# fkluger/vanishing_points_2017

Measured on AMD Instinct MI355X. Metric: images/sec (LSD->CNN->EM) + horizon-AUC parity, YUD-shape, 1/2/4/8 GPU, higher is better.
Workload: dtype f32 (CNN: f32 operands / accumulation / results; conv1 multiply EXACT bf16 pieces of the f32 operands (three per operand) on the bf16 matrix cores; conv2-5, fc6 and fc7 multiply scaled fp16 PAIRS of the f32 operands (22 of 24 significand bits, three exact products per f32 product) on the fp16 matrix

## Files before the change

vanishing_points_2017_amd/csrc/em_run.hpp:

```cpp
#ifndef VPK_EM_RUN_HPP_
#define VPK_EM_RUN_HPP_

#include "em_ctx.hpp"
#include "em_linalg.hpp"
#include "em_setup.hpp"
#include "em_estep.hpp"
#include "em_smooth.hpp"
#include "em_assign.hpp"
#include "em_mstep.hpp"
#include "em_vpset.hpp"

namespace vpk {

struct EmOut {
    double* vp;
    double* sigma;
    double* counts;
    double* counts_w;
    int* num_vp;
    long long* assoc;
    int* iterations;
    int* status;
    unsigned* flags;
    double* metric;
// ... 63 lines not shown
        *o.status = status;
        *o.flags = sh.flags;
    }
    block_sync();
}

VPK_DEV void trace_put(EmOut& o, int i, int slot, double v) {
    if (o.trace && tid() == 0) o.trace[TRACE_COLS * i + slot] = v;
}
VPK_DEV void trace_add(EmOut& o, int i, int slot, double v) {
    if (o.trace && tid() == 0) o.trace[TRACE_COLS * i + slot] += v;
}


constexpr int EM_DONE = 0, EM_SUSPENDED = 1;
constexpr long long EM_NO_DEADLINE = 0x7fffffffffffffffll;
struct EmSlice {
    long long deadline;
    int start_iter;
};

VPK_DEVFN void save_state(EmCtx& c) {
    typedef VPK_GLOBAL unsigned long long* gup;
    gup dst = (gup)c.state;
    const unsigned long long* src = reinterpret_cast<const unsigned long long*>(&SH());
    for (int q = tid(); q < (int)(sizeof(Shared) / 8); q += nthreads()) dst[q] = src[q];
    block_sync();
}
VPK_DEVFN void restore_state(EmCtx& c) {
    typedef const VPK_GLOBAL unsigned long long* cgup;
    cgup src = (cgup)c.state;
    unsigned long long* dst = reinterpret_cast<unsigned long long*>(&SH());
    block_sync();
    for (int q = tid(); q < (int)(sizeof(Shared) / 8); q += nthreads()) dst[q] = src[q];
    block_sync();
}

template <int MEASURE = VPK_DIST_ANGLE>
VPK_DEVFN int em_run(EmCtx& c, EmOut& o, EmSlice& sl) {
    static_assert(MEASURE == VPK_DIST_ANGLE || MEASURE == VPK_DIST_DOTPROD, "the EM runs \"angle\" and \"dotprod\" (vp_localisation.py:196-203)");
    Shared& sh = SH();
    const vpk_em_params& P = c.prm;
    const double max_stdd = MEASURE == VPK_DIST_DOTPROD ? 1e-3 : 1e-6;
    const double merge_thresh_final = P.merge_thresh * 10;
    const int split_merge_it = 100;
    long long tk = clock_ticks();
    const long long t_begin = tk;
    int first = 0;
    bool ew_valid = false;
    if (sl.start_iter >= 0) {
        restore_state(c);
        first = sl.start_iter;
    } else {
    if (tid() == 0) { sh.flags = 0; sh.M = 0; sh.ncomp = 0; sh.ibuf[5] = 0; sh.ibuf[2] = 0; sh.active_us = 0; for (int q = 8; q < 16; ++q) sh.dbuf[q] = 0; }
    block_sync();
    if (o.trace)
        for (int q = tid(); q < TRACE_COLS * (P.num_iter + 1); q += nthreads()) o.trace[q] = 0.0;
    if (c.N <= 0) { write_result(c, o, VPK_EM_NO_VP, 0); return EM_DONE; }

    if (P.use_weights) { pairwise_setup(c, true); zero_tail_rows(c); }
    else pairwise_setup(c, false);
    trace_put(o, P.num_iter, 0, lap(tk));
    normalise_lines(c);
    for (int q = tid(); q < 3 * c.N; q += nthreads()) c.lcopy[q] = c.l[q];
    for (int q = tid(); q < 4 * c.N; q += nthreads()) c.lpcopy[q] = c.lp[q];
    block_sync();
    c.l = c.lcopy;
    c.lp = c.lpcopy;
    initial_vps(c);
    const int m_found = sh.M;
    prior_setup(c);
    if (m_found == 0) { write_result(c, o, VPK_EM_NO_INITIAL_VP, 0); return EM_DONE; }
    if (c.init_vp) {
        if (tid() == 0) {
            int m = c.n_init < MAXM ? c.n_init : MAXM;
            for (int k = 0; k < m; ++k) {
                cgdp q = c.init_vp + 3 * (size_t)k;
                double nr = norm3(q[0], q[1], q[2]);
                sh.cur[3 * k] = q[0] / nr; sh.cur[3 * k + 1] = q[1] / nr; sh.cur[3 * k + 2] = q[2] / nr;
            }
            sh.M = m;
        }
        block_sync();
    }
    weights_setup(c);
    line_geometry_setup<MEASURE>(c);
    for (int m = tid(); m < MAXM; m += nthreads()) {
        sh.s[m] = 1.0 * (sh.sigma_prior * max_stdd);
        sh.nxt[3 * m] = 0; sh.nxt[3 * m + 1] = 0; sh.nxt[3 * m + 2] = 0;
    }
    block_sync();

    estep<MEASURE>(c, sh.cur);
    smooth(c);
    assign_lines<MEASURE>(c, true);
    count_lines(c);
    const int m_initial = sh.M;
    for (int m = tid(); m < sh.M; m += nthreads()) sh.removed[m] = sh.cnt[m] < 3;
    block_sync();
    compact_vps(c);
    ew_valid = c.smoother != 1 && sh.M == m_initial;
    trace_put(o, P.num_iter, 1, lap(tk));
    }

    for (int i = first; i < P.num_iter; ++i) {
        if (sl.deadline != EM_NO_DEADLINE && i > sl.start_iter) {
            if (tid() == 0) sh.ibuf[6] = clock_ticks() >= sl.deadline;
            block_sync();
            if (sh.ibuf[6]) {
                if (tid() == 0) sh.active_us += (double)(clock_ticks() - t_begin) * CLOCK_US;
                block_sync();
                save_state(c);
                sl.start_iter = i;
                return EM_SUSPENDED;
            }
        }
        tk = clock_ticks();
        const long long t_iter = tk;
        if (sh.M == 0) { write_result(c, o, VPK_EM_NO_VP, 0); return EM_DONE; }
        double events = 0;
        bool ew_skip = ew_valid;
        ew_valid = false;
        if (i % P.split_merge_freq == 0 && i > 0 && i < split_merge_it && P.do_split) {
            int mb = sh.M;
// ... 111 lines not shown
```

vanishing_points_2017_amd/csrc/em_setup.hpp:

```cpp
#ifndef VPK_EM_SETUP_HPP_
#define VPK_EM_SETUP_HPP_

#include "em_ctx.hpp"

namespace vpk {

VPK_DEVFN void normalise_lines(EmCtx& c) {
    for (int n = tid(); n < c.N; n += nthreads()) {
        gdp r = c.l + 3 * (size_t)n;
        for (int pass = 0; pass < 2; ++pass) {
            double nr = norm3(r[0], r[1], r[2]);
            r[0] /= nr; r[1] /= nr; r[2] /= nr;
        }
    }
    block_sync();
}

constexpr int PW_TILED_MIN = 512;
constexpr int PW_RB = 16;
constexpr int PW_TLD = WAVE + 1;
constexpr int PW_TBUF = 2 * PW_RB * PW_TLD;
VPK_DEV void pairwise_tiles(EmCtx& c) {
    const int N = c.N;
    double* gs = SCRATCH() + wave_id() * (PW_RB * 10);
    static_assert(8 * PW_RB * 10 <= PART_DOUBLES, "row geometries of eight waves in the setup scratch");
    const bool tbuf_ok = WAVE == 64 && PART_DOUBLES + nwaves() * PW_TBUF <= c.wt_doubles;
    double* tb = SCRATCH() + PART_DOUBLES + wave_id() * PW_TBUF;
    const int nb = (N + PW_RB - 1) / PW_RB;
    int t = 0;
    for (int I = 0; I < nb; ++I) {
        const int i0 = I * PW_RB;
        const int ilast = (i0 + PW_RB < N ? i0 + PW_RB : N) - 1;
        const int nch = (ilast + WAVE - 1) / WAVE;
        for (int jc = 0; jc < nch; ++jc, ++t) {
            if (t % nwaves() != wave_id()) continue;
            if (lane() < PW_RB) {
                const int i = i0 + lane() < N ? i0 + lane() : N - 1;
                double a[4];
#pragma unroll
                for (int q = 0; q < 4; ++q) a[q] = c.lp[4 * (size_t)i + q];
                const LineGeom g = line_geom(a);
                double* o = gs + lane() * 10;
                o[0] = g.x1; o[1] = g.y1; o[2] = g.x2; o[3] = g.y2; o[4] = g.dx; o[5] = g.dy; o[6] = g.nn; o[7] = g.vx; o[8] = g.vy; o[9] = g.nv;
            }
            wave_lds_order();
            const int j = jc * WAVE + lane();
            const int jj = j < N ? j : N - 1;
            double b[4];
#pragma unroll
            for (int q = 0; q < 4; ++q) b[q] = c.lp[4 * (size_t)jj + q];
            const LineGeom gb = line_geom(b);
            auto row_geom = [&](int r) {
                const double* o = gs + r * 10;
                LineGeom g;
                g.x1 = o[0]; g.y1 = o[1]; g.x2 = o[2]; g.y2 = o[3]; g.dx = o[4]; g.dy = o[5]; g.nn = o[6]; g.vx = o[7]; g.vy = o[8]; g.nv = o[9];
                return g;
            };
            auto put = [&](int i, double d, double sim) {
                if (!(j < i && i < N)) return;
                c.lsim[(size_t)i * c.ld + j] = sim;
                c.lsim[(size_t)j * c.ld + i] = sim;
                c.pdist[(size_t)i * c.ld + j] = d;
                c.pdist[(size_t)j * c.ld + i] = d;
            };
            const bool interior = tbuf_ok && jc * WAVE + WAVE - 1 < i0 && i0 + PW_RB <= N;
            for (int r = 0; r < PW_RB; r += 2) {
                const LineGeom g0 = row_geom(r), g1 = row_geom(r + 1);
                const double d0 = line_distance_closest(g0, gb);
                const double d1 = line_distance_closest(g1, gb);
                const double s0 = lines_cosangle(g0, gb, 9.0) * proximity(d0, g0.nv, gb.nv, 1.0);
                const double s1 = lines_cosangle(g1, gb, 9.0) * proximity(d1, g1.nv, gb.nv, 1.0);
                if (interior) {
                    c.lsim[(size_t)(i0 + r) * c.ld + j] = s0;   c.pdist[(size_t)(i0 + r) * c.ld + j] = d0;
                    c.lsim[(size_t)(i0 + r + 1) * c.ld + j] = s1; c.pdist[(size_t)(i0 + r + 1) * c.ld + j] = d1;
                    tb[r * PW_TLD + lane()] = s0;               tb[(PW_RB + r) * PW_TLD + lane()] = d0;
                    tb[(r + 1) * PW_TLD + lane()] = s1;         tb[(PW_RB + r + 1) * PW_TLD + lane()] = d1;
                } else {
                    put(i0 + r, d0, s0);
                    put(i0 + r + 1, d1, s1);
                }
            }
            wave_lds_order();
            if (interior) {
                const int cp = lane() & 7, jr = lane() >> 3;
#pragma unroll
                for (int q = 0; q < 8; ++q) {
                    const int jl = 8 * q + jr;
                    const size_t at = (size_t)(jc * WAVE + jl) * c.ld + i0 + 2 * cp;
                    store_cols2(c.lsim + at, tb[(2 * cp) * PW_TLD + jl], tb[(2 * cp + 1) * PW_TLD + jl]);
                    store_cols2(c.pdist + at, tb[(PW_RB + 2 * cp) * PW_TLD + jl], tb[(PW_RB + 2 * cp + 1) * PW_TLD + jl]);
                }
                wave_lds_order();
            }
        }
    }
    for (int i = tid(); i < N; i += nthreads()) {
        c.lsim[(size_t)i * c.ld + i] = 0.0;
        c.pdist[(size_t)i * c.ld + i] = 4.0;
    }
}

VPK_DEVFN void pairwise_setup(EmCtx& c, bool want_lsim) {
    const int N = c.N;
    if (want_lsim) {
        if (N >= PW_TILED_MIN && WAVE == 64 && c.smoother != 1) pairwise_tiles(c);
        else
        for (int r = wave_id(); 2 * r < N; r += nwaves()) {
            const int i0 = r, i1 = N - 1 - r;
            const int len = i0 == i1 ? i0 : i0 + i1;
            double a0[4], a1[4];
#pragma unroll
            for (int q = 0; q < 4; ++q) { a0[q] = c.lp[4 * (size_t)i0 + q]; a1[q] = c.lp[4 * (size_t)i1 + q]; }
            const LineGeom g0 = line_geom(a0), g1 = line_geom(a1);
            auto one = [&](int t, double& d, double& sim) {
                const bool first = t < i0;
                const int j = t < len ? (first ? t : t - i0) : 0;
                const LineGeom& ga = first ? g0 : g1;
                double b[4] = {c.lp[4 * (size_t)j], c.lp[4 * (size_t)j + 1], c.lp[4 * (size_t)j + 2], c.lp[4 * (size_t)j + 3]};
                const LineGeom gb = line_geom(b);
                d = line_distance_closest(ga, gb);
                sim = lines_cosangle(ga, gb, 9.0) * proximity(d, ga.nv, gb.nv, 1.0);
            };
            auto put = [&](int t, double d, double sim) {
                if (t >= len) return;
                const int i = t < i0 ? i0 : i1, j = t < i0 ? t : t - i0;
                c.lsim[(size_t)i * c.ld + j] = sim;
                c.lsim[(size_t)j * c.ld + i] = sim;
                c.pdist[(size_t)i * c.ld + j] = d;
                c.pdist[(size_t)j * c.ld + i] = d;
            };
            for (int t = lane(); t < len; t += 2 * WAVE) {
                double d0, s0, d1, s1;
                one(t, d0, s0);
                one(t + WAVE, d1, s1);
                put(t, d0, s0);
                put(t + WAVE, d1, s1);
            }
            if (lane() == 0) {
                c.lsim[(size_t)i0 * c.ld + i0] = 0.0;
                c.pdist[(size_t)i0 * c.ld + i0] = 4.0;
                c.lsim[(size_t)i1 * c.ld + i1] = 0.0;
                c.pdist[(size_t)i1 * c.ld + i1] = 4.0;
            }
        }
        block_sync();
        for (int i = wave_id(); i < N; i += nwaves()) {
            cgdp srow = c.lsim + (size_t)i * c.ld;
            double rsum = 0.0;
            for (int j = lane(); j < N; j += WAVE) rsum += srow[j];
            rsum = wave_sum(rsum);
            if (lane() == 0) c.rowsum[i] = rsum;
        }
        constexpr int RPW = WAVE / ROWG;
        const int grp = lane() / ROWG, gl = lane() % ROWG;
        const int k1 = N < KNN1 ? N : KNN1;
        const int k2 = N < KNN2 ? N : KNN2;
        double* ks = SCRATCH() + (wave_id() * RPW + grp) * (4 * KNN1 + KNN2);
        for (int base = wave_id() * RPW; base < N; base += nwaves() * RPW) {
            const int i = base + grp;
            const bool valid = i < N;
            const int ii = valid ? i : 0;
            double td[KNN1];
            int tj[KNN1];
#pragma unroll
            for (int q = 0; q < KNN1; ++q) { td[q] = 1e300; tj[q] = 0x7fffffff; }
            cgdp drow = c.pdist + (size_t)ii * c.ld;
            for (int j0 = gl; j0 < N; j0 += 4 * ROWG) {
                double dv[4];
#pragma unroll
                for (int u = 0; u < 4; ++u) dv[u] = (j0 + u * ROWG < N) ? drow[j0 + u * ROWG] : 1e300;
#pragma unroll
                for (int u = 0; u < 4; ++u) {
                    double nd = dv[u];
                    int nj = (j0 + u * ROWG < N) ? j0 + u * ROWG : 0x7fffffff;
#pragma unroll
                    for (int q = 0; q < KNN1; ++q) {
                        const bool lt = (nd < td[q]) || (nd == td[q] && nj < tj[q]);
                        const double od = td[q];
                        const int oj = tj[q];
                        td[q] = lt ? nd : od;
                        tj[q] = lt ? nj : oj;
                        nd = lt ? od : nd;
                        nj = lt ? oj : nj;
                    }
                }
            }
            for (int r = 0; r < k1; ++r) {
                double bd = td[0];
                int bj = tj[0];
                row16_argmin(bd, bj);
                if (tj[0] == bj && td[0] == bd) {
#pragma unroll
                    for (int q = 0; q + 1 < KNN1; ++q) { td[q] = td[q + 1]; tj[q] = tj[q + 1]; }
                    td[KNN1 - 1] = 1e300;
                    tj[KNN1 - 1] = 0x7fffffff;
                }
                if (gl == 0) { ks[r] = (double)bj; ks[KNN1 + r] = bd; }
            }
            wave_sync();
            double a[4] = {c.lp[4 * (size_t)ii], c.lp[4 * (size_t)ii + 1], c.lp[4 * (size_t)ii + 2], c.lp[4 * (size_t)ii + 3]};
            const double len_a = norm2(a[0] - a[2], a[1] - a[3]);
            for (int q = gl; q < k1; q += ROWG) {
                int j = (int)ks[q];
                j = (valid && j >= 0 && j < N) ? j : 0;
                double b[4] = {c.lp[4 * (size_t)j], c.lp[4 * (size_t)j + 1], c.lp[4 * (size_t)j + 2], c.lp[4 * (size_t)j + 3]};
                ks[2 * KNN1 + q] = lines_cosangle(a, b, 9.0);
                const double dq = j == ii ? line_distance_closest(a, b) : ks[KNN1 + q];
                ks[3 * KNN1 + q] = proximity(dq, len_a, line_length(b), 1.0);
            }
            wave_sync();
            for (int q = gl; q < k1; q += ROWG) {
                const double cq = ks[2 * KNN1 + q];
                int rank = 0;
                for (int p = 0; p < k1; ++p) {
                    const double cp = ks[2 * KNN1 + p];
                    rank += (cp > cq) || (cp == cq && p > q);
                }
                if (rank < k2) ks[4 * KNN1 + rank] = ks[3 * KNN1 + q] * cq;
            }
            wave_sync();
            if (gl == 0 && valid) {
                double sum = 0.0;
                for (int r = 0; r < k2; ++r) sum += ks[4 * KNN1 + r];
                c.lscore[i] = sum / k2;
                c.langle[i] = line_angle(a);
            }
            wave_sync();
        }
        block_sync();
        return;
    }
    double* ks = SCRATCH() + wave_id() * (4 * KNN1 + KNN2);
    const int k1 = N < KNN1 ? N : KNN1;
    const int k2 = N < KNN2 ? N : KNN2;
    for (int i = wave_id(); i < N; i += nwaves()) {
        double a[4] = {c.lp[4 * (size_t)i], c.lp[4 * (size_t)i + 1], c.lp[4 * (size_t)i + 2],
                       c.lp[4 * (size_t)i + 3]};
        const LineGeom ga = line_geom(a);
        const double len_a = ga.nv;
        double rsum = 0.0;
        double td[KNN1];
        int tj[KNN1];
#pragma unroll
        for (int q = 0; q < KNN1; ++q) { td[q] = 1e300; tj[q] = 0x7fffffff; }
        auto pair_eval = [&](int j, double& d, double& sim) {
            const int jj = j < N ? j : i;
            double b[4] = {c.lp[4 * (size_t)jj], c.lp[4 * (size_t)jj + 1], c.lp[4 * (size_t)jj + 2],
                           c.lp[4 * (size_t)jj + 3]};
            const LineGeom gb = line_geom(b);
            d = line_distance_closest(ga, gb);
            sim = want_lsim ? lines_cosangle(ga, gb, 9.0) * proximity(d, len_a, gb.nv, 1.0) : 0.0;
        };
        auto pair_commit = [&](int j, double d, double sim) {
            if (j >= N) return;
            if (want_lsim) {
                sim = (i == j) ? 0.0 : sim;
                c.lsim[(size_t)i * c.ld + j] = sim;
                rsum += sim;
            }
            double nd = (i == j) ? 4.0 : d;
            int nj = j;
#pragma unroll
            for (int q = 0; q < KNN1; ++q) {
                const bool lt = (nd < td[q]) || (nd == td[q] && nj < tj[q]);
                const double od = td[q];
                const int oj = tj[q];
                td[q] = lt ? nd : od;
                tj[q] = lt ? nj : oj;
                nd = lt ? od : nd;
                nj = lt ? oj : nj;
            }
        };
        for (int j = lane(); j < N; j += 2 * WAVE) {
            double d0, s0, d1, s1;
            pair_eval(j, d0, s0);
            pair_eval(j + WAVE, d1, s1);
            pair_commit(j, d0, s0);
            pair_commit(j + WAVE, d1, s1);
        }
        rsum = wave_sum(rsum);
        if (lane() == 0) c.rowsum[i] = rsum;
        for (int r = 0; r < k1; ++r) {
// ... 9 lines not shown
            if (lane() == 0) { ks[r] = (double)bj; ks[KNN1 + r] = bd; }
        }
        wave_sync();
        for (int q = lane(); q < k1; q += WAVE) {
            int j = (int)ks[q];
            double b[4] = {c.lp[4 * (size_t)j], c.lp[4 * (size_t)j + 1], c.lp[4 * (size_t)j + 2],
                           c.lp[4 * (size_t)j + 3]};
            ks[2 * KNN1 + q] = lines_cosangle(a, b, 9.0);
            const double dq = j == i ? line_distance_closest(a, b) : ks[KNN1 + q];
            ks[3 * KNN1 + q] = proximity(dq, len_a, line_length(b), 1.0);
        }
        wave_sync();
        for (int q = lane(); q < k1; q += WAVE) {
            const double cq = ks[2 * KNN1 + q];
            int rank = 0;
            for (int p = 0; p < k1; ++p) {
                const double cp = ks[2 * KNN1 + p];
                rank += (cp > cq) || (cp == cq && p > q);
            }
            if (rank < k2) ks[4 * KNN1 + rank] = ks[3 * KNN1 + q] * cq;
        }
        wave_sync();
        if (lane() == 0) {
            double sum = 0.0;
            for (int r = 0; r < k2; ++r) sum += ks[4 * KNN1 + r];
            c.lscore[i] = sum / k2;
            c.langle[i] = line_angle(a);
        }
        wave_sync();
    }
    block_sync();
}

VPK_DEVFN void weights_setup(EmCtx& c) {
    const int N = c.N;
    const bool uw = c.prm.use_weights != 0;
    for (int n = tid(); n < N; n += nthreads()) {
        double a[4] = {c.lp[4 * (size_t)n], c.lp[4 * (size_t)n + 1], c.lp[4 * (size_t)n + 2],
                       c.lp[4 * (size_t)n + 3]};
        c.lweight[n] = uw ? line_length(a) * clip(c.lscore[n], 0.2, 1.0) : 1.0;
    }
    block_sync();
    for (int k = tid(); k < N; k += nthreads()) {
        c.den[k] = 1 + c.prm.wbias * c.lweight[k] * (uw ? c.rowsum[k] : 0.0);
        if (uw && !(fabs(c.rowsum[k]) <= 1.7976931348623157e308)) SH().ibuf[2] = 1;
    }
    block_sync();
}

VPK_DEVFN void prior_setup(EmCtx& c) {
    Shared& sh = SH();
    float* keep = (float*)SCRATCH();
    if (tid() == 0) sh.sigma_prior = PI_D / (1.282 * GRIDN);
    prior_keep_sum(c.cnn, sh.wts, keep);
    {
        const float sum = keep[NCELL];
        const float dv = prior_norm_f32(sh.sigma_prior);
        int* wcount = (int*)(SCRATCH() + 256);
        for (int base = 0; base < NCELL; base += nthreads()) {
            const int i = base + tid();
            float w = 0.f;
            if (i < NCELL) w = prior_weight(keep[i], sum, dv);
            const unsigned long long pos = wave_ballot(i < NCELL && w > 0);
            if (lane() == 0) wcount[wave_id()] = popcount64(pos);
            block_sync();
            int before = (base == 0) ? 0 : sh.ncomp;
            for (int k = 0; k < wave_id(); ++k) before += wcount[k];
            const int nc = before + popcount64(pos & lanes_below());
            if (i < NCELL) {
                sh.wts[i] = w;
                if (w > 0 && nc < MAXCOMP) {
                    sh.pma[nc] = grid_centre(i % GRIDN);
                    sh.pmb[nc] = grid_centre(i / GRIDN);
                    sh.pw[nc] = (double)w;
                }
            }
            block_sync();
            if (tid() == 0) {
                int tot = before;
                for (int k = 0; k < nwaves(); ++k) tot += wcount[k];
                sh.ncomp = tot < MAXCOMP ? tot : MAXCOMP;
            }
            block_sync();
        }
    }
}

VPK_DEVFN void initial_vps(EmCtx& c) {
    Shared& sh = SH();
    cgfp r = c.cnn;
    for (int i = tid(); i < NCELL; i += nthreads()) {
        int b = i / GRIDN, a = i % GRIDN;
        float vm = r[i];
        float vu = (a + 1 < GRIDN) ? r[b * GRIDN + a + 1] : 0.f;
        float vd = (a - 1 > 0) ? r[b * GRIDN + a - 1] : 0.f;
        float vl = (b - 1 > 0) ? r[(b - 1) * GRIDN + a] : 0.f;
        float vr = (b + 1 < GRIDN) ? r[(b + 1) * GRIDN + a] : 0.f;
        sh.mx[i] = (vm > vu && vm > vd && vm > vl && vm > vr) ? 1 : 0;
    }
    block_sync();
    unsigned char* keep = (unsigned char*)SCRATCH();
    double* cand = SCRATCH() + 64;
    const int num_max = c.prm.num_init_vp;
    for (int i = tid(); i < NCELL; i += nthreads()) {
        int k = 0;
        if (sh.mx[i]) {
            int rank = 0;
            float vi = r[i];
            for (int j = 0; j < NCELL; ++j)
                if (sh.mx[j]) rank += (r[j] > vi) || (r[j] == vi && j > i);
            k = rank < num_max;
        }
        keep[i] = (unsigned char)k;
        cand[4 * i + 3] = 0.0;
    }
    block_sync();
    const int S = c.ssize;
    for (int cell = wave_id(); cell < NCELL; cell += nwaves()) {
        if (!keep[cell]) continue;
        int ra = cell / GRIDN, rb = cell % GRIDN;
        int r0 = ra * S / GRIDN, r1 = (ra + 1) * S / GRIDN;
        int c0 = rb * S / GRIDN, c1 = (rb + 1) * S / GRIDN;
        int bw = c1 - c0, npix = (r1 - r0) * bw;
        constexpr int PV = 10;
        int mxv = 0, cntp = 0, sr = 0, sc = 0;
        if (npix <= PV * WAVE) {
            int vals[PV];
#pragma unroll
            for (int q = 0; q < PV; ++q) {
                const int p = lane() + q * WAVE;
                const int pc = p < npix ? p : 0;
                const int v = c.sphere[(size_t)(S - 1 - (r0 + pc / bw)) * S + c0 + pc % bw];
                vals[q] = p < npix ? v : -1;
            }
#pragma unroll
            for (int q = 0; q < PV; ++q) mxv = vals[q] > mxv ? vals[q] : mxv;
            mxv = wave_max_int(mxv);
            if (mxv == 0) continue;
#pragma unroll
            for (int q = 0; q < PV; ++q) {
                const int p = lane() + q * WAVE;
                if (vals[q] == mxv) { ++cntp; sr += p / bw; sc += p % bw; }
            }
        } else {
            for (int p = lane(); p < npix; p += WAVE) {
                int rr = r0 + p / bw, cc = c0 + p % bw;
                int v = c.sphere[(size_t)(S - 1 - rr) * S + cc];
                mxv = v > mxv ? v : mxv;
            }
            mxv = wave_max_int(mxv);
            if (mxv == 0) continue;
            for (int p = lane(); p < npix; p += WAVE) {
                int rr = p / bw, cc = p % bw;
                int v = c.sphere[(size_t)(S - 1 - (r0 + rr)) * S + c0 + cc];
                if (v == mxv) { ++cntp; sr += rr; sc += cc; }
            }
        }
        cntp = wave_sum_int(cntp);
        sr = wave_sum_int(sr);
        sc = wave_sum_int(sc);
        if (lane() == 0) {
            double avg_r = (double)sr / cntp, avg_c = (double)sc / cntp;
            double ia = avg_c + c0, ib = avg_r + r0;
            double alpha = (ia - 0.5 * S + 0.5) * PI_D / S;
            double beta = (ib - 0.5 * S + 0.5) * PI_D / S;
            double px = sin(alpha) * cos(beta), py = sin(beta), pz = cos(alpha) * cos(beta);
            double sg = sign_np(pz);
            cand[4 * cell + 0] = px * sg;
            cand[4 * cell + 1] = py * sg;
            cand[4 * cell + 2] = pz * sg;
            cand[4 * cell + 3] = 1.0;
        }
    }
    block_sync();
    if (tid() == 0) {
        int m = 0;
        for (int cell = 0; cell < NCELL; ++cell) {
            if (cand[4 * cell + 3] != 0.0 && m < MAXM) {
                sh.cur[3 * m + 0] = cand[4 * cell + 0];
                sh.cur[3 * m + 1] = cand[4 * cell + 1];
                sh.cur[3 * m + 2] = cand[4 * cell + 2];
                ++m;
            }
        }
        sh.M = m;
    }
    block_sync();
}

template <int MEASURE = VPK_DIST_ANGLE>
VPK_DEVFN void line_geometry_setup(EmCtx& c) {
    for (int n = tid(); n < c.N; n += nthreads()) {
        if (MEASURE == VPK_DIST_DOTPROD) {
            cgdp q = c.l + 3 * (size_t)n;
            c.drow[n] = q[0];
            c.drow[(size_t)c.ldn + n] = q[1];
            c.drow[2 * (size_t)c.ldn + n] = q[2];
            continue;
        }
        cgdp q = c.lp + 4 * (size_t)n;
        if (MEASURE == VPK_DIST_AREA) {
            const double mx = 0.5 * (q[0] + q[2]), my = 0.5 * (q[1] + q[3]);
            c.drow[n] = mx;
            c.drow[(size_t)c.ldn + n] = my;
            c.drow[2 * (size_t)c.ldn + n] = q[0];
            c.drow[3 * (size_t)c.ldn + n] = q[1];
            c.drow[4 * (size_t)c.ldn + n] = norm2(mx - q[2], my - q[3]);
            continue;
        }
        const double v2x = q[0] - q[2], v2y = q[1] - q[3];
        c.drow[n] = 0.5 * (q[0] + q[2]);
        c.drow[(size_t)c.ldn + n] = 0.5 * (q[1] + q[3]);
        c.drow[2 * (size_t)c.ldn + n] = v2x;
        c.drow[3 * (size_t)c.ldn + n] = v2y;
        c.drow[4 * (size_t)c.ldn + n] = norm2(v2x, v2y);
    }
    block_sync();
}

}
#endif
```

vanishing_points_2017_amd/csrc/prior_device.hpp:

```cpp
#ifndef VPK_PRIOR_DEVICE_HPP_
#define VPK_PRIOR_DEVICE_HPP_

#include "wave_prims.hpp"

namespace vpk {

constexpr int GRIDN = 20;
constexpr int NCELL = GRIDN * GRIDN;
constexpr int MAXCOMP = 100;
constexpr double PI_D = 3.141592653589793238462643383279502884;

VPK_DEV bool is_nan(double x) { return x != x; }
VPK_DEV double exp_underflow(double x) { return x < -746.0 ? 0.0 : exp(x); }

VPK_DEV void vp_angles(double x0, double x1, double& alpha, double& beta) {
    beta = asin(x1);
    double inner = x0 / cos(beta);
    inner = inner < 1 ? inner : (is_nan(inner) ? inner : 1.0);
    inner = inner > -1 ? inner : (is_nan(inner) ? inner : -1.0);
    alpha = asin(inner);
}

VPK_DEV double mixture_term(double alpha, double beta, double ma, double mb, double kk) {
    double d1 = (alpha - ma) * (alpha - ma) + (beta - mb) * (beta - mb);
    double d2 = (alpha - ma + PI_D) * (alpha - ma + PI_D) + (beta + mb) * (beta + mb);
    double d3 = (alpha - ma - PI_D) * (alpha - ma - PI_D) + (beta + mb) * (beta + mb);
    double d4 = (alpha + ma) * (alpha + ma) + (beta - mb - PI_D) * (beta - mb - PI_D);
    double e4 = exp_underflow(d4 * kk);
    return (((exp_underflow(d1 * kk) + exp_underflow(d2 * kk)) + exp_underflow(d3 * kk)) + e4) + e4;
}

VPK_DEV float np_pairwise_block_f32(const float* a, int n) {
    float r[8];
    for (int j = 0; j < 8; ++j) r[j] = a[j];
    int i;
    for (i = 8; i < n - (n % 8); i += 8)
        for (int j = 0; j < 8; ++j) r[j] += a[i + j];
    float res = ((r[0] + r[1]) + (r[2] + r[3])) + ((r[4] + r[5]) + (r[6] + r[7]));
    for (; i < n; ++i) res += a[i];
    return res;
}
VPK_DEV float np_pairwise_sum_f32_400(const float* a) {
    float lo = np_pairwise_block_f32(a, 96) + np_pairwise_block_f32(a + 96, 104);
    float hi = np_pairwise_block_f32(a + 200, 96) + np_pairwise_block_f32(a + 296, 104);
    return lo + hi;
}

VPK_DEV double grid_centre(int i) {
    double start = -(GRIDN - 1.0) / GRIDN * PI_D / 2;
    double stop = (GRIDN - 1.0) / GRIDN * PI_D / 2;
    double step = (stop - start) / (GRIDN - 1);
    return i == GRIDN - 1 ? stop : i * step + start;
}

VPK_DEV void prior_keep_sum(cgfp cnn, float* wts, float* keep) {
    for (int i = tid(); i < NCELL; i += nthreads()) wts[i] = cnn[i];
    block_sync();
    for (int i = tid(); i < NCELL; i += nthreads()) {
        float wi = wts[i];
        int rank = 0;
        for (int j = 0; j < NCELL; ++j) {
            float wj = wts[j];
            rank += (wj > wi) || (wj == wi && j > i);
        }
        keep[i] = rank < MAXCOMP ? wi : 0.f;
    }
    block_sync();
    if (tid() == 0) keep[NCELL] = np_pairwise_sum_f32_400(keep);
    block_sync();
}
VPK_DEV float prior_norm_f32(double sigma) { return (float)(2 * PI_D * sigma * sigma); }
VPK_DEV float prior_weight(float kept, float sum, float dv) {
    float w = kept / sum;
    return w / dv;
}

constexpr int PRIOR_TILE = WAVE;
constexpr int PRIOR_CHUNK = 128;
constexpr size_t PRIOR_LDS_BYTES = 3 * PRIOR_CHUNK * sizeof(double);

struct MixtureArgs {
    int ncomp, npts;
    cgdp means;
    long long means_stride;
    cgdp weights;
    double kk;
    cgdp pts;
    long long pts_stride;
    gdp angles_out;
    gdp pdf_out;
};

template <int DIM> VPK_DEV void mixture_pdf_tile(const MixtureArgs& a, int b, int t) {
    double* sma = reinterpret_cast<double*>(lds_base());
    double* smb = sma + PRIOR_CHUNK;
    double* sw = smb + PRIOR_CHUNK;
    const int i = t * PRIOR_TILE + tid();
    const bool live = i < a.npts;
    double alpha = 0.0, beta = 0.0;
    if (live) {
        cgdp p = a.pts + (size_t)b * a.pts_stride + (size_t)i * DIM;
        if (DIM == 3) vp_angles(p[0], p[1], alpha, beta);
        else { alpha = p[0]; beta = p[1]; }
    }
    cgdp mean = a.means + (size_t)b * a.means_stride;
    cgdp wt = a.weights + (size_t)b * a.ncomp;
    double acc = 0.0;
    for (int c0 = 0; c0 < a.ncomp; c0 += PRIOR_CHUNK) {
        const int nc = a.ncomp - c0 < PRIOR_CHUNK ? a.ncomp - c0 : PRIOR_CHUNK;
        block_sync();
        for (int q = tid(); q < nc; q += nthreads()) {
            sma[q] = mean[2 * (size_t)(c0 + q)];
            smb[q] = mean[2 * (size_t)(c0 + q) + 1];
            sw[q] = wt[c0 + q];
        }
        block_sync();
        if (live)
            for (int q = 0; q < nc; ++q) {
                const double w = sw[q];
                if (!(w > 0)) continue;
                acc += mixture_term(alpha, beta, sma[q], smb[q], a.kk) * w;
// ... 14 lines not shown
```

Before: 22970.

## Parallelise EM setup: threshold kNN, tabled line geometry, block-parallel initial VPs

```diff
diff --git a/vanishing_points_2017_amd/csrc/em_knn.hpp b/vanishing_points_2017_amd/csrc/em_knn.hpp
--- /dev/null
+++ b/vanishing_points_2017_amd/csrc/em_knn.hpp
@@ -0,0 +1,62 @@
+#ifndef VPK_EM_KNN_HPP_
+#define VPK_EM_KNN_HPP_
+
+#ifndef VPK_DEV
+#define VPK_DEV static inline
+#endif
+
+namespace vpk {
+namespace knn {
+
+constexpr double SENT_D = 1e300;
+constexpr int SENT_J = 0x7fffffff;
+constexpr int CAP = 28;
+constexpr int CAND_DOUBLES = CAP + CAP / 2;
+
+VPK_DEV bool key_less(double ad, int aj, double bd, int bj) { return (ad < bd) || (ad == bd && aj < bj); }
+
+VPK_DEV void key_of(double d, int j, int n, double& kd, int& kj) {
+    const bool ok = j < n && d <= SENT_D;
+    kd = ok ? d : SENT_D;
+    kj = ok ? j : SENT_J;
+}
+
+struct Top2 {
+    double d0, d1;
+    int j0, j1;
+};
+VPK_DEV void top2_init(Top2& t) { t.d0 = t.d1 = SENT_D; t.j0 = t.j1 = SENT_J; }
+VPK_DEV void top2_push(Top2& t, double kd, int kj) {
+    const bool lt0 = key_less(kd, kj, t.d0, t.j0);
+    const bool lt1 = key_less(kd, kj, t.d1, t.j1);
+    t.d1 = lt0 ? t.d0 : (lt1 ? kd : t.d1);
+    t.j1 = lt0 ? t.j0 : (lt1 ? kj : t.j1);
+    t.d0 = lt0 ? kd : t.d0;
+    t.j0 = lt0 ? kj : t.j0;
+}
+VPK_DEV void top2_pop_if(Top2& t, double bd, int bj) {
+    const bool won = t.j0 == bj && t.d0 == bd;
+    t.d0 = won ? t.d1 : t.d0;
+    t.j0 = won ? t.j1 : t.j0;
+    t.d1 = won ? SENT_D : t.d1;
+    t.j1 = won ? SENT_J : t.j1;
+}
+
+VPK_DEV bool is_candidate(double kd, int kj, double td, int tj) {
+    return kj != SENT_J && !key_less(td, tj, kd, kj);
+}
+VPK_DEV int cand_slot(unsigned bits, int g, int listed) { return listed + __builtin_popcount(bits & ((1u << g) - 1u)); }
+
+VPK_DEV void rank_and_place(int g, int G, int cnt, const double* cd, const int* cj, int k, double* out_j, double* out_d) {
+    for (int q = g; q < cnt; q += G) {
+        const double dq = cd[q];
+        const int jq = cj[q];
+        int rank = 0;
+        for (int p = 0; p < cnt; ++p) rank += key_less(cd[p], cj[p], dq, jq) ? 1 : 0;
+        if (rank < k) { out_j[rank] = (double)jq; out_d[rank] = dq; }
+    }
+}
+
+}
+}
+#endif
diff --git a/vanishing_points_2017_amd/csrc/em_run.hpp b/vanishing_points_2017_amd/csrc/em_run.hpp
--- a/vanishing_points_2017_amd/csrc/em_run.hpp
+++ b/vanishing_points_2017_amd/csrc/em_run.hpp
@@ -139,7 +139,7 @@
         restore_state(c);
         first = sl.start_iter;
     } else {
-    if (tid() == 0) { sh.flags = 0; sh.M = 0; sh.ncomp = 0; sh.ibuf[5] = 0; sh.ibuf[2] = 0; sh.active_us = 0; for (int q = 8; q < 16; ++q) sh.dbuf[q] = 0; }
+    if (tid() == 0) { sh.flags = 0; sh.M = 0; sh.ncomp = 0; sh.ibuf[5] = 0; sh.ibuf[2] = 0; sh.active_us = 0; sh.dbuf[0] = 0; sh.dbuf[1] = 0; for (int q = 8; q < 16; ++q) sh.dbuf[q] = 0; }
     block_sync();
     if (o.trace)
         for (int q = tid(); q < TRACE_COLS * (P.num_iter + 1); q += nthreads()) o.trace[q] = 0.0;
@@ -148,15 +148,20 @@
     if (P.use_weights) { pairwise_setup(c, true); zero_tail_rows(c); }
     else pairwise_setup(c, false);
     trace_put(o, P.num_iter, 0, lap(tk));
+    trace_put(o, P.num_iter, 10, sh.dbuf[0]);
+    trace_put(o, P.num_iter, 11, sh.dbuf[1]);
     normalise_lines(c);
     for (int q = tid(); q < 3 * c.N; q += nthreads()) c.lcopy[q] = c.l[q];
     for (int q = tid(); q < 4 * c.N; q += nthreads()) c.lpcopy[q] = c.lp[q];
     block_sync();
     c.l = c.lcopy;
     c.lp = c.lpcopy;
+    long long tq = clock_ticks();
     initial_vps(c);
+    trace_put(o, 0, 8, lap(tq));
     const int m_found = sh.M;
     prior_setup(c);
+    trace_put(o, 0, 9, lap(tq));
     if (m_found == 0) { write_result(c, o, VPK_EM_NO_INITIAL_VP, 0); return EM_DONE; }
     if (c.init_vp) {
         if (tid() == 0) {
diff --git a/vanishing_points_2017_amd/csrc/em_setup.hpp b/vanishing_points_2017_amd/csrc/em_setup.hpp
--- a/vanishing_points_2017_amd/csrc/em_setup.hpp
+++ b/vanishing_points_2017_amd/csrc/em_setup.hpp
@@ -2,6 +2,7 @@
 #define VPK_EM_SETUP_HPP_
 
 #include "em_ctx.hpp"
+#include "em_knn.hpp"
 
 namespace vpk {
 
@@ -100,11 +101,181 @@
     }
 }
 
+template <bool B> struct BoolTag { static constexpr bool value = B; };
+VPK_DEV LineGeom line_geom_known(const double a[4], double nn, double nv) {
+    LineGeom g;
+    g.x1 = a[0]; g.y1 = a[1]; g.x2 = a[2]; g.y2 = a[3];
+    g.dx = a[2] - a[0]; g.dy = a[3] - a[1];
+    g.nn = nn;
+    g.vx = a[0] - a[2]; g.vy = a[1] - a[3];
+    g.nv = nv;
+    return g;
+}
+
+VPK_DEV void knn_by_insertion(cgdp drow, int N, int gl, int k1, double* ks) {
+    double td[KNN1];
+    int tj[KNN1];
+#pragma unroll
+    for (int q = 0; q < KNN1; ++q) { td[q] = 1e300; tj[q] = 0x7fffffff; }
+    for (int j0 = gl; j0 < N; j0 += 4 * ROWG) {
+        double dv[4];
+#pragma unroll
+        for (int u = 0; u < 4; ++u) dv[u] = (j0 + u * ROWG < N) ? drow[j0 + u * ROWG] : 1e300;
+#pragma unroll
+        for (int u = 0; u < 4; ++u) {
+            double nd = dv[u];
+            int nj = (j0 + u * ROWG < N) ? j0 + u * ROWG : 0x7fffffff;
+#pragma unroll
+            for (int q = 0; q < KNN1; ++q) {
+                const bool lt = (nd < td[q]) || (nd == td[q] && nj < tj[q]);
+                const double od = td[q];
+                const int oj = tj[q];
+                td[q] = lt ? nd : od;
+                tj[q] = lt ? nj : oj;
+                nd = lt ? od : nd;
+                nj = lt ? oj : nj;
+            }
+        }
+    }
+    for (int r = 0; r < k1; ++r) {
+        double bd = td[0];
+        int bj = tj[0];
+        row16_argmin(bd, bj);
+        if (tj[0] == bj && td[0] == bd) {
+#pragma unroll
+            for (int q = 0; q + 1 < KNN1; ++q) { td[q] = td[q + 1]; tj[q] = tj[q + 1]; }
+            td[KNN1 - 1] = 1e300;
+            tj[KNN1 - 1] = 0x7fffffff;
+        }
+        if (gl == 0) { ks[r] = (double)bj; ks[KNN1 + r] = bd; }
+    }
+}
+
+constexpr int KNN_RPW = WAVE / ROWG;
+constexpr int KS_ROW = 2 * KNN1 + (2 * KNN1 + KNN2 > knn::CAND_DOUBLES ? 2 * KNN1 + KNN2 : knn::CAND_DOUBLES);
+static_assert(WAVE != 64 || 8 * KNN_RPW * KS_ROW <= PART_DOUBLES, "kNN rows of eight waves in the setup scratch");
+VPK_DEV double* knn_row_scratch() { return SCRATCH() + (wave_id() * KNN_RPW + lane() / ROWG) * KS_ROW; }
+VPK_DEV bool knn_by_threshold(cgdp drow, int N, int k1) {
+    const int grp = lane() / ROWG, gl = lane() % ROWG;
+    double* ks = knn_row_scratch();
+    for (int q = gl; q < k1; q += ROWG) { ks[q] = (double)knn::SENT_J; ks[KNN1 + q] = knn::SENT_D; }
+    constexpr int KB = 16;
+    const bool one_trip = N <= KB * ROWG;
+    double dv[KB];
+    knn::Top2 t2;
+    knn::top2_init(t2);
+    for (int jb = 0; jb < N; jb += KB * ROWG) {
+#pragma unroll
+        for (int u = 0; u < KB; ++u) { const int j = jb + u * ROWG + gl; dv[u] = j < N ? drow[j] : knn::SENT_D; }
+#pragma unroll
+        for (int u = 0; u < KB; ++u) {
+            double kd;
+            int kj;
+            knn::key_of(dv[u], jb + u * ROWG + gl, N, kd, kj);
+            knn::top2_push(t2, kd, kj);
+        }
+    }
+    double taud = knn::SENT_D;
+    int tauj = knn::SENT_J;
+    for (int r = 0; r < k1; ++r) {
+        taud = t2.d0;
+        tauj = t2.j0;
+        row16_argmin(taud, tauj);
+        knn::top2_pop_if(t2, taud, tauj);
+    }
+    double* cd = ks + 2 * KNN1;
+    int* cj = (int*)(cd + knn::CAP);
+    int cnt = 0;
+    for (int jb = 0; jb < N; jb += KB * ROWG) {
+        if (!one_trip) {
+#pragma unroll
+            for (int u = 0; u < KB; ++u) { const int j = jb + u * ROWG + gl; dv[u] = j < N ? drow[j] : knn::SENT_D; }
+        }
+#pragma unroll
+        for (int u = 0; u < KB; ++u) {
+            if (jb + u * ROWG >= N) break;
+            double kd;
+            int kj;
+            knn::key_of(dv[u], jb + u * ROWG + gl, N, kd, kj);
+            const bool in = knn::is_candidate(kd, kj, taud, tauj);
+            const unsigned bits = (unsigned)(wave_ballot(in) >> (grp * ROWG)) & ((1u << ROWG) - 1u);
+            const int at = knn::cand_slot(bits, gl, cnt);
+            if (in && at < knn::CAP) { cd[at] = kd; cj[at] = kj; }
+            cnt += popcount64(bits);
+        }
+    }
+    wave_sync();
+    if (cnt > knn::CAP) return false;
+    knn::rank_and_place(gl, ROWG, cnt, cd, cj, k1, ks, ks + KNN1);
+    return true;
+}
+
+VPK_DEV void line_rating_rows(EmCtx& c) {
+    const int N = c.N;
+    constexpr int RPW = KNN_RPW;
+    const int grp = lane() / ROWG, gl = lane() % ROWG;
+    const int k1 = N < KNN1 ? N : KNN1;
+    const int k2 = N < KNN2 ? N : KNN2;
+    double* ks = knn_row_scratch();
+    for (int base = wave_id() * RPW; base < N; base += nwaves() * RPW) {
+        const int i = base + grp;
+        const bool valid = i < N;
+        const int ii = valid ? i : 0;
+        cgdp drow = c.pdist + (size_t)ii * c.ld;
+        const bool insertion = c.smoother == 1 || !knn_by_threshold(drow, N, k1);
+        if (insertion) knn_by_insertion(drow, N, gl, k1, ks);
+        wave_sync();
+        double a[4] = {c.lp[4 * (size_t)ii], c.lp[4 * (size_t)ii + 1], c.lp[4 * (size_t)ii + 2], c.lp[4 * (size_t)ii + 3]};
+        const double len_a = norm2(a[0] - a[2], a[1] - a[3]);
+        for (int q = gl; q < k1; q += ROWG) {
+            int j = (int)ks[q];
+            j = (valid && j >= 0 && j < N) ? j : 0;
+            double b[4] = {c.lp[4 * (size_t)j], c.lp[4 * (size_t)j + 1], c.lp[4 * (size_t)j + 2], c.lp[4 * (size_t)j + 3]};
+            ks[2 * KNN1 + q] = lines_cosangle(a, b, 9.0);
+            const double dq = j == ii ? line_distance_closest(a, b) : ks[KNN1 + q];
+            ks[3 * KNN1 + q] = proximity(dq, len_a, line_length(b), 1.0);
+        }
+        wave_sync();
+        for (int q = gl; q < k1; q += ROWG) {
+            const double cq = ks[2 * KNN1 + q];
+            int rank = 0;
+            for (int p = 0; p < k1; ++p) {
+                const double cp = ks[2 * KNN1 + p];
+                rank += (cp > cq) || (cp == cq && p > q);
+            }
+            if (rank < k2) ks[4 * KNN1 + rank] = ks[3 * KNN1 + q] * cq;
+        }
+        wave_sync();
+        if (gl == 0 && valid) {
+            double sum = 0.0;
+            for (int r = 0; r < k2; ++r) sum += ks[4 * KNN1 + r];
+            c.lscore[i] = sum / k2;
+            c.langle[i] = line_angle(a);
+        }
+        wave_sync();
+    }
+}
+
 VPK_DEVFN void pairwise_setup(EmCtx& c, bool want_lsim) {
     const int N = c.N;
     if (want_lsim) {
+        long long tq_ = clock_ticks();
         if (N >= PW_TILED_MIN && WAVE == 64 && c.smoother != 1) pairwise_tiles(c);
-        else
+        else {
+        const bool geo_lds = c.smoother != 1 && 2 * N <= PART_DOUBLES;
+        double* gnn = SCRATCH();
+        double* gnv = SCRATCH() + N;
+        if (geo_lds) {
+            for (int n = tid(); n < N; n += nthreads()) {
+                double a[4] = {c.lp[4 * (size_t)n], c.lp[4 * (size_t)n + 1], c.lp[4 * (size_t)n + 2], c.lp[4 * (size_t)n + 3]};
+                const LineGeom g = line_geom(a);
+                gnn[n] = g.nn;
+                gnv[n] = g.nv;
+            }
+            block_sync();
+        }
+        auto rows = [&](auto from_table) {
+        constexpr bool TAB = decltype(from_table)::value;
         for (int r = wave_id(); 2 * r < N; r += nwaves()) {
             const int i0 = r, i1 = N - 1 - r;
             const int len = i0 == i1 ? i0 : i0 + i1;
@@ -117,7 +288,7 @@
                 const int j = t < len ? (first ? t : t - i0) : 0;
                 const LineGeom& ga = first ? g0 : g1;
                 double b[4] = {c.lp[4 * (size_t)j], c.lp[4 * (size_t)j + 1], c.lp[4 * (size_t)j + 2], c.lp[4 * (size_t)j + 3]};
-                const LineGeom gb = line_geom(b);
+                const LineGeom gb = TAB ? line_geom_known(b, gnn[j], gnv[j]) : line_geom(b);
                 d = line_distance_closest(ga, gb);
                 sim = lines_cosangle(ga, gb, 9.0) * proximity(d, ga.nv, gb.nv, 1.0);
             };
@@ -143,91 +314,50 @@
                 c.pdist[(size_t)i1 * c.ld + i1] = 4.0;
             }
         }
+        };
+        if (geo_lds) rows(BoolTag<true>());
+        else rows(BoolTag<false>());
+        }
         block_sync();
-        for (int i = wave_id(); i < N; i += nwaves()) {
-            cgdp srow = c.lsim + (size_t)i * c.ld;
-            double rsum = 0.0;
-            for (int j = lane(); j < N; j += WAVE) rsum += srow[j];
-            rsum = wave_sum(rsum);
-            if (lane() == 0) c.rowsum[i] = rsum;
-        }
-        constexpr int RPW = WAVE / ROWG;
-        const int grp = lane() / ROWG, gl = lane() % ROWG;
-        const int k1 = N < KNN1 ? N : KNN1;
-        const int k2 = N < KNN2 ? N : KNN2;
-        double* ks = SCRATCH() + (wave_id() * RPW + grp) * (4 * KNN1 + KNN2);
-        for (int base = wave_id() * RPW; base < N; base += nwaves() * RPW) {
-            const int i = base + grp;
-            const bool valid = i < N;
-            const int ii = valid ? i : 0;
-            double td[KNN1];
-            int tj[KNN1];
-#pragma unroll
-            for (int q = 0; q < KNN1; ++q) { td[q] = 1e300; tj[q] = 0x7fffffff; }
-            cgdp drow = c.pdist + (size_t)ii * c.ld;
-            for (int j0 = gl; j0 < N; j0 += 4 * ROWG) {
-                double dv[4];
-#pragma unroll
-                for (int u = 0; u < 4; ++u) dv[u] = (j0 + u * ROWG < N) ? drow[j0 + u * ROWG] : 1e300;
-#pragma unroll
-                for (int u = 0; u < 4; ++u) {
-                    double nd = dv[u];
-                    int nj = (j0 + u * ROWG < N) ? j0 + u * ROWG : 0x7fffffff;
-#pragma unroll
-                    for (int q = 0; q < KNN1; ++q) {
-                        const bool lt = (nd < td[q]) || (nd == td[q] && nj < tj[q]);
-                        const double od = td[q];
-                        const int oj = tj[q];
-                        td[q] = lt ? nd : od;
-                        tj[q] = lt ? nj : oj;
-                        nd = lt ? od : nd;
-                        nj = lt ? oj : nj;
+        if (tid() == 0) SH().dbuf[0] = lap(tq_);
+        if (c.smoother == 1) {
+            for (int i = wave_id(); i < N; i += nwaves()) {
+                cgdp srow = c.lsim + (size_t)i * c.ld;
+                double rsum = 0.0;
+                for (int j = lane(); j < N; j += WAVE) rsum += srow[j];
+                rsum = wave_sum(rsum);
+                if (lane() == 0) c.rowsum[i] = rsum;
+            }
+        } else {
+            constexpr int RS_ROWS = 4, RS_COLS = 8;
+            for (int i0 = wave_id() * RS_ROWS; i0 < N; i0 += nwaves() * RS_ROWS) {
+                double rs[RS_ROWS];
+#pragma unroll
+                for (int q = 0; q < RS_ROWS; ++q) rs[q] = 0.0;
+                for (int jb = 0; jb < N; jb += RS_COLS * WAVE) {
+                    double v[RS_ROWS][RS_COLS];
+#pragma unroll
+                    for (int q = 0; q < RS_ROWS; ++q) {
+                        cgdp srow = c.lsim + (size_t)(i0 + q < N ? i0 + q : N - 1) * c.ld;
+#pragma unroll
+                        for (int u = 0; u < RS_COLS; ++u) { const int j = jb + u * WAVE + lane(); v[q][u] = j < N ? srow[j] : 0.0; }
                     }
+#pragma unroll
+                    for (int q = 0; q < RS_ROWS; ++q)
+#pragma unroll
+                        for (int u = 0; u < RS_COLS; ++u)
+                            if (jb + u * WAVE + lane() < N) rs[q] += v[q][u];
                 }
-            }
-            for (int r = 0; r < k1; ++r) {
-                double bd = td[0];
-                int bj = tj[0];
-                row16_argmin(bd, bj);
-                if (tj[0] == bj && td[0] == bd) {
-#pragma unroll
-                    for (int q = 0; q + 1 < KNN1; ++q) { td[q] = td[q + 1]; tj[q] = tj[q + 1]; }
-                    td[KNN1 - 1] = 1e300;
-                    tj[KNN1 - 1] = 0x7fffffff;
+#pragma unroll
+                for (int q = 0; q < RS_ROWS; ++q) {
+                    const double rsum = wave_sum(rs[q]);
+                    if (lane() == 0 && i0 + q < N) c.rowsum[i0 + q] = rsum;
                 }
-                if (gl == 0) { ks[r] = (double)bj; ks[KNN1 + r] = bd; }
-            }
-            wave_sync();
-            double a[4] = {c.lp[4 * (size_t)ii], c.lp[4 * (size_t)ii + 1], c.lp[4 * (size_t)ii + 2], c.lp[4 * (size_t)ii + 3]};
-            const double len_a = norm2(a[0] - a[2], a[1] - a[3]);
-            for (int q = gl; q < k1; q += ROWG) {
-                int j = (int)ks[q];
-                j = (valid && j >= 0 && j < N) ? j : 0;
-                double b[4] = {c.lp[4 * (size_t)j], c.lp[4 * (size_t)j + 1], c.lp[4 * (size_t)j + 2], c.lp[4 * (size_t)j + 3]};
-                ks[2 * KNN1 + q] = lines_cosangle(a, b, 9.0);
-                const double dq = j == ii ? line_distance_closest(a, b) : ks[KNN1 + q];
-                ks[3 * KNN1 + q] = proximity(dq, len_a, line_length(b), 1.0);
-            }
-            wave_sync();
-            for (int q = gl; q < k1; q += ROWG) {
-                const double cq = ks[2 * KNN1 + q];
-                int rank = 0;
-                for (int p = 0; p < k1; ++p) {
-                    const double cp = ks[2 * KNN1 + p];
-                    rank += (cp > cq) || (cp == cq && p > q);
-                }
-                if (rank < k2) ks[4 * KNN1 + rank] = ks[3 * KNN1 + q] * cq;
-            }
-            wave_sync();
-            if (gl == 0 && valid) {
-                double sum = 0.0;
-                for (int r = 0; r < k2; ++r) sum += ks[4 * KNN1 + r];
-                c.lscore[i] = sum / k2;
-                c.langle[i] = line_angle(a);
-            }
-            wave_sync();
-        }
+            }
+        }
+        line_rating_rows(c);
         block_sync();
+        if (tid() == 0) SH().dbuf[1] = lap(tq_);
         return;
     }
     double* ks = SCRATCH() + wave_id() * (4 * KNN1 + KNN2);
@@ -343,7 +473,7 @@
     Shared& sh = SH();
     float* keep = (float*)SCRATCH();
     if (tid() == 0) sh.sigma_prior = PI_D / (1.282 * GRIDN);
-    prior_keep_sum(c.cnn, sh.wts, keep);
+    prior_keep_sum(c.cnn, sh.wts, keep, c.smoother == 1);
     {
         const float sum = keep[NCELL];
         const float dv = prior_norm_f32(sh.sigma_prior);
@@ -377,7 +507,64 @@
     }
 }
 
-VPK_DEVFN void initial_vps(EmCtx& c) {
+VPK_DEV void initial_vp_of_cell(EmCtx& c, int cell, double* out) {
+    const int S = c.ssize;
+    int ra = cell / GRIDN, rb = cell % GRIDN;
+    int r0 = ra * S / GRIDN, r1 = (ra + 1) * S / GRIDN;
+    int c0 = rb * S / GRIDN, c1 = (rb + 1) * S / GRIDN;
+    int bw = c1 - c0, npix = (r1 - r0) * bw;
+    constexpr int PV = 10;
+    int mxv = 0, cntp = 0, sr = 0, sc = 0;
+    if (npix <= PV * WAVE) {
+        int vals[PV];
+#pragma unroll
+        for (int q = 0; q < PV; ++q) {
+            const int p = lane() + q * WAVE;
+            const int pc = p < npix ? p : 0;
+            const int v = c.sphere[(size_t)(S - 1 - (r0 + pc / bw)) * S + c0 + pc % bw];
+            vals[q] = p < npix ? v : -1;
+        }
+#pragma unroll
+        for (int q = 0; q < PV; ++q) mxv = vals[q] > mxv ? vals[q] : mxv;
+        mxv = wave_max_int(mxv);
+        if (mxv == 0) return;
+#pragma unroll
+        for (int q = 0; q < PV; ++q) {
+            const int p = lane() + q * WAVE;
+            if (vals[q] == mxv) { ++cntp; sr += p / bw; sc += p % bw; }
+        }
+    } else {
+        for (int p = lane(); p < npix; p += WAVE) {
+            int rr = r0 + p / bw, cc = c0 + p % bw;
+            int v = c.sphere[(size_t)(S - 1 - rr) * S + cc];
+            mxv = v > mxv ? v : mxv;
+        }
+        mxv = wave_max_int(mxv);
+        if (mxv == 0) return;
+        for (int p = lane(); p < npix; p += WAVE) {
+            int rr = p / bw, cc = p % bw;
+            int v = c.sphere[(size_t)(S - 1 - (r0 + rr)) * S + c0 + cc];
+            if (v == mxv) { ++cntp; sr += rr; sc += cc; }
+        }
+    }
+    cntp = wave_sum_int(cntp);
+    sr = wave_sum_int(sr);
+    sc = wave_sum_int(sc);
+    if (lane() == 0) {
+        double avg_r = (double)sr / cntp, avg_c = (double)sc / cntp;
+        double ia = avg_c + c0, ib = avg_r + r0;
+        double alpha = (ia - 0.5 * S + 0.5) * PI_D / S;
+        double beta = (ib - 0.5 * S + 0.5) * PI_D / S;
+        double px = sin(alpha) * cos(beta), py = sin(beta), pz = cos(alpha) * cos(beta);
+        double sg = sign_np(pz);
+        out[0] = px * sg;
+        out[1] = py * sg;
+        out[2] = pz * sg;
+        out[3] = 1.0;
+    }
+}
+
+VPK_DEV void initial_vps_serial(EmCtx& c) {
     Shared& sh = SH();
     cgfp r = c.cnn;
     for (int i = tid(); i < NCELL; i += nthreads()) {
@@ -406,63 +593,8 @@
         cand[4 * i + 3] = 0.0;
     }
     block_sync();
-    const int S = c.ssize;
-    for (int cell = wave_id(); cell < NCELL; cell += nwaves()) {
-        if (!keep[cell]) continue;
-        int ra = cell / GRIDN, rb = cell % GRIDN;
-        int r0 = ra * S / GRIDN, r1 = (ra + 1) * S / GRIDN;
-        int c0 = rb * S / GRIDN, c1 = (rb + 1) * S / GRIDN;
-        int bw = c1 - c0, npix = (r1 - r0) * bw;
-        constexpr int PV = 10;
-        int mxv = 0, cntp = 0, sr = 0, sc = 0;
-        if (npix <= PV * WAVE) {
-            int vals[PV];
-#pragma unroll
-            for (int q = 0; q < PV; ++q) {
-                const int p = lane() + q * WAVE;
-                const int pc = p < npix ? p : 0;
-                const int v = c.sphere[(size_t)(S - 1 - (r0 + pc / bw)) * S + c0 + pc % bw];
-                vals[q] = p < npix ? v : -1;
-            }
-#pragma unroll
-            for (int q = 0; q < PV; ++q) mxv = vals[q] > mxv ? vals[q] : mxv;
-            mxv = wave_max_int(mxv);
-            if (mxv == 0) continue;
-#pragma unroll
-            for (int q = 0; q < PV; ++q) {
-                const int p = lane() + q * WAVE;
-                if (vals[q] == mxv) { ++cntp; sr += p / bw; sc += p % bw; }
-            }
-        } else {
-            for (int p = lane(); p < npix; p += WAVE) {
-                int rr = r0 + p / bw, cc = c0 + p % bw;
-                int v = c.sphere[(size_t)(S - 1 - rr) * S + cc];
-                mxv = v > mxv ? v : mxv;
-            }
-            mxv = wave_max_int(mxv);
-            if (mxv == 0) continue;
-            for (int p = lane(); p < npix; p += WAVE) {
-                int rr = p / bw, cc = p % bw;
-                int v = c.sphere[(size_t)(S - 1 - (r0 + rr)) * S + c0 + cc];
-                if (v == mxv) { ++cntp; sr += rr; sc += cc; }
-            }
-        }
-        cntp = wave_sum_int(cntp);
-        sr = wave_sum_int(sr);
-        sc = wave_sum_int(sc);
-        if (lane() == 0) {
-            double avg_r = (double)sr / cntp, avg_c = (double)sc / cntp;
-            double ia = avg_c + c0, ib = avg_r + r0;
-            double alpha = (ia - 0.5 * S + 0.5) * PI_D / S;
-            double beta = (ib - 0.5 * S + 0.5) * PI_D / S;
-            double px = sin(alpha) * cos(beta), py = sin(beta), pz = cos(alpha) * cos(beta);
-            double sg = sign_np(pz);
-            cand[4 * cell + 0] = px * sg;
-            cand[4 * cell + 1] = py * sg;
-            cand[4 * cell + 2] = pz * sg;
-            cand[4 * cell + 3] = 1.0;
-        }
-    }
+    for (int cell = wave_id(); cell < NCELL; cell += nwaves())
+        if (keep[cell]) initial_vp_of_cell(c, cell, cand + 4 * cell);
     block_sync();
     if (tid() == 0) {
         int m = 0;
@@ -476,6 +608,96 @@
         }
         sh.M = m;
     }
+    block_sync();
+}
+
+VPK_DEV int block_position_of_flagged(bool flag, int* wcount, int& total) {
+    const unsigned long long b = wave_ballot(flag);
+    if (lane() == 0) wcount[wave_id()] = popcount64(b);
+    block_sync();
+    int before = 0, tot = 0;
+    for (int k = 0; k < nwaves(); ++k) {
+        const int n = wcount[k];
+        before += k < wave_id() ? n : 0;
+        tot += n;
+    }
+    block_sync();
+    total = tot;
+    return before + popcount64(b & lanes_below());
+}
+
+VPK_DEVFN void initial_vps(EmCtx& c) {
+    if (c.smoother == 1) { initial_vps_serial(c); return; }
+    Shared& sh = SH();
+    cgfp r = c.cnn;
+    double* cand = SCRATCH();
+    float* mv = (float*)(SCRATCH() + 4 * NCELL);
+    unsigned short* mi = (unsigned short*)(SCRATCH() + 4 * NCELL + NCELL / 2);
+    unsigned short* kl = mi + NCELL;
+    int* wcount = (int*)(kl + NCELL);
+    static_assert(4 * NCELL + NCELL / 2 + NCELL / 4 + NCELL / 4 + 16 <= PART_DOUBLES, "lists of initial_vps in the setup scratch");
+    int nm = 0;
+    for (int base = 0; base < NCELL; base += nthreads()) {
+        const int i = base + tid();
+        bool ismax = false;
+        float vm = 0.f;
+        if (i < NCELL) {
+            int b = i / GRIDN, a = i % GRIDN;
+            vm = r[i];
+            float vu = (a + 1 < GRIDN) ? r[b * GRIDN + a + 1] : 0.f;
+            float vd = (a - 1 > 0) ? r[b * GRIDN + a - 1] : 0.f;
+            float vl = (b - 1 > 0) ? r[(b - 1) * GRIDN + a] : 0.f;
+            float vr = (b + 1 < GRIDN) ? r[(b + 1) * GRIDN + a] : 0.f;
+            ismax = vm > vu && vm > vd && vm > vl && vm > vr;
+        }
+        int tot;
+        const int at = nm + block_position_of_flagged(ismax, wcount, tot);
+        if (ismax) { mv[at] = vm; mi[at] = (unsigned short)i; }
+        nm += tot;
+    }
+    block_sync();
+    const int num_max = c.prm.num_init_vp;
+    int nk = 0;
+    for (int base = 0; base < NCELL; base += nthreads()) {
+        const int q = base + tid();
+        bool kept = false;
+        int i = 0;
+        if (q < nm) {
+            int rank = 0;
+            const float vi = mv[q];
+            i = mi[q];
+            for (int k0 = 0; k0 < nm; k0 += 4) {
+                float v[4];
+                int j[4];
+#pragma unroll
+                for (int u = 0; u < 4; ++u) { const int k = k0 + u < nm ? k0 + u : nm - 1; v[u] = mv[k]; j[u] = mi[k]; }
+#pragma unroll
+                for (int u = 0; u < 4; ++u) rank += (k0 + u < nm) && ((v[u] > vi) || (v[u] == vi && j[u] > i));
+            }
+            kept = rank < num_max;
+        }
+        int tot;
+        const int at = nk + block_position_of_flagged(kept, wcount, tot);
+        if (kept) { kl[at] = (unsigned short)i; cand[4 * at + 3] = 0.0; }
+        nk += tot;
+    }
+    block_sync();
+    for (int q = wave_id(); q < nk; q += nwaves()) initial_vp_of_cell(c, kl[q], cand + 4 * q);
+    block_sync();
+    int m = 0;
+    for (int base = 0; base < NCELL; base += nthreads()) {
+        const int q = base + tid();
+        const bool found = q < nk && cand[4 * (q < nk ? q : 0) + 3] != 0.0;
+        int tot;
+        const int at = m + block_position_of_flagged(found, wcount, tot);
+        if (found && at < MAXM) {
+            sh.cur[3 * at + 0] = cand[4 * q + 0];
+            sh.cur[3 * at + 1] = cand[4 * q + 1];
+            sh.cur[3 * at + 2] = cand[4 * q + 2];
+        }
+        m += tot;
+    }
+    if (tid() == 0) sh.M = m < MAXM ? m : MAXM;
     block_sync();
 }
 
diff --git a/vanishing_points_2017_amd/csrc/prior_device.hpp b/vanishing_points_2017_amd/csrc/prior_device.hpp
--- a/vanishing_points_2017_amd/csrc/prior_device.hpp
+++ b/vanishing_points_2017_amd/csrc/prior_device.hpp
@@ -53,20 +53,53 @@
     return i == GRIDN - 1 ? stop : i * step + start;
 }
 
-VPK_DEV void prior_keep_sum(cgfp cnn, float* wts, float* keep) {
+VPK_DEV float np_pairwise_sum_f32_400_wave(const float* a) {
+    const int blk = (lane() >> 3) & 3, j = lane() & 7;
+    const int base = blk == 0 ? 0 : (blk == 1 ? 96 : (blk == 2 ? 200 : 296));
+    const int n = (blk & 1) ? 104 : 96;
+    float r = a[base + j];
+    for (int i = 8; i < n; i += 8) r += a[base + i + j];
+    float b[4];
+#pragma unroll
+    for (int q = 0; q < 4; ++q) {
+        float t[8];
+#pragma unroll
+        for (int u = 0; u < 8; ++u) t[u] = (float)wave_bcast((double)r, 8 * q + u);
+        b[q] = ((t[0] + t[1]) + (t[2] + t[3])) + ((t[4] + t[5]) + (t[6] + t[7]));
+    }
+    return (b[0] + b[1]) + (b[2] + b[3]);
+}
+
+VPK_DEV void prior_keep_sum(cgfp cnn, float* wts, float* keep, bool serial = false) {
     for (int i = tid(); i < NCELL; i += nthreads()) wts[i] = cnn[i];
     block_sync();
     for (int i = tid(); i < NCELL; i += nthreads()) {
         float wi = wts[i];
         int rank = 0;
-        for (int j = 0; j < NCELL; ++j) {
-            float wj = wts[j];
-            rank += (wj > wi) || (wj == wi && j > i);
+        if (serial) {
+            for (int j = 0; j < NCELL; ++j) {
+                float wj = wts[j];
+                rank += (wj > wi) || (wj == wi && j > i);
+            }
+        } else {
+            static_assert(NCELL % 8 == 0, "eight cells per trip");
+            for (int j0 = 0; j0 < NCELL; j0 += 8) {
+                float wj[8];
+#pragma unroll
+                for (int u = 0; u < 8; ++u) wj[u] = wts[j0 + u];
+#pragma unroll
+                for (int u = 0; u < 8; ++u) rank += (wj[u] > wi) || (wj[u] == wi && j0 + u > i);
+            }
         }
         keep[i] = rank < MAXCOMP ? wi : 0.f;
     }
     block_sync();
-    if (tid() == 0) keep[NCELL] = np_pairwise_sum_f32_400(keep);
+    if (serial || WAVE != 64) {
+        if (tid() == 0) keep[NCELL] = np_pairwise_sum_f32_400(keep);
+    } else if (wave_id() == 0) {
+        const float sum = np_pairwise_sum_f32_400_wave(keep);
+        if (lane() == 0) keep[NCELL] = sum;
+    }
     block_sync();
 }
 VPK_DEV float prior_norm_f32(double sigma) { return (float)(2 * PI_D * sigma * sigma); }
```

After: 23330, median of 5. 1.5% higher.
